# ivpml84079/Probabilistic-Self-Update-Line-Vector-Set-Based-Point-Cloud-Registration

Hardware: NVIDIA B200
Metric: registrations/s (higher is better)
Workload: dtype f64+f32

## Files before the change

probabilistic-self-update-line-vector-set-based-point-cloud-registration_b200/csrc/engine.cu:

```cuda
#include <cuda_runtime.h>
#include <sched.h>

#include <algorithm>
#include <atomic>
#include <chrono>
#if defined(__SSE2__)
#include <emmintrin.h>
#endif
#include <cmath>
#include <cstdlib>
#include <cstring>
#include <condition_variable>
#include <deque>
#include <functional>
#include <map>
#include <memory>
#include <mutex>
#include <string>
#include <thread>
#include <utility>
#include <vector>

#include "common.cuh"
#include "engine.cuh"
// ... 621 lines not shown
    PSU_CUDA(cudaEventRecord(ev_begin, st));
  }
  PSU_CUDA(cudaMemsetAsync(m.border, 0, sizeof(unsigned long long) * (size_t)B, st));
  PSU_CUDA(cudaMemsetAsync(m.n_done, 0, sizeof(int) * 4, st));
  PSU_CUDA(cudaMemcpyAsync(m.k1, k1.data(), sizeof(K1Job) * (size_t)B, cudaMemcpyHostToDevice, st));
  PSU_CUDA(cudaMemcpyAsync(m.cj, cj.data(), sizeof(CompactJob) * (size_t)B, cudaMemcpyHostToDevice, st));
  PSU_CUDA(cudaMemcpyAsync(m.pj, pj.data(), sizeof(PackJob) * (size_t)2 * B, cudaMemcpyHostToDevice, st));

  if (ratio) {
    if (int rc = ratio_count(st, rj, m.rj, maxC, [&](size_t bytes) -> void* { return d_hist.ensure(bytes) ? nullptr : d_hist.p; },
                             ev_m0, ev_m1))
      return rc;
    launches += 8;
  } else {
    {
      dim3 grid((unsigned)((maxC + 255) / 256), (unsigned)(2 * B));
      engine_pack_kernel<<<grid, 256, 0, st>>>(m.pj);
      PSU_CHECK_LAUNCH("engine_pack_kernel");
      ++launches;
    }
    PSU_CUDA(cudaEventRecord(ev_m0, st));
    if (!sharded || row_e > row_b)
      if (int rc = launch_consistency_mask(st, m.k1, B, maxC, sharded ? row_e - row_b : maxC, true)) return rc;
    PSU_CUDA(cudaEventRecord(ev_m1, st));
    ++launches;
    if (int rc = launch_compact_edges(st, m.cj, B, maxC, true, false, false)) return rc;
    ++launches;
  }
  if (int rc = h_small.ensure((sizeof(unsigned long long) + sizeof(int)) * (size_t)B + 64 + 66 * sizeof(unsigned long long)))
    return rc;
  unsigned long long* h_nedges = reinterpret_cast<unsigned long long*>(h_small.p);
  volatile int* h_done = reinterpret_cast<volatile int*>(reinterpret_cast<char*>(h_small.p) + sizeof(unsigned long long) * (size_t)B);
  unsigned long long* h_counts = reinterpret_cast<unsigned long long*>(
      reinterpret_cast<char*>(h_small.p) + align_up((sizeof(unsigned long long) + sizeof(int)) * (size_t)B + 16, 16));
  std::vector<unsigned long long> shard_off;
  if (sharded) {
    if (int rc = comm_allgather_u64(comm, st, m.n_edges, m.counts_all)) return rc;
    PSU_CUDA(cudaMemcpyAsync(h_counts, m.counts_all, sizeof(unsigned long long) * (size_t)comm_world(comm),
                             cudaMemcpyDeviceToHost, st));
    PSU_CUDA(cudaStreamSynchronize(st));
    shard_off.assign((size_t)comm_world(comm) + 1, 0ull);
    for (int r = 0; r < comm_world(comm); ++r) shard_off[(size_t)r + 1] = shard_off[(size_t)r] + h_counts[r];
    h_nedges[0] = shard_off.back();
    PSU_CUDA(cudaMemcpyAsync(m.n_edges, h_nedges, sizeof(unsigned long long), cudaMemcpyHostToDevice, st));
  } else {
    PSU_CUDA(cudaMemcpyAsync(h_nedges, m.n_edges, sizeof(unsigned long long) * (size_t)B, cudaMemcpyDeviceToHost, st));
    PSU_CUDA(cudaStreamSynchronize(st));
  }

  bool narrow = !sharded && !debug_knobs().edge_wide;
  for (int b = 0; b < B; ++b) narrow = narrow && edge_narrow_fits(lay[(size_t)(b0 + b)].Ccap);
  const int grid_ctas_max = sm_count() / (B > 0 ? B : 1);
  unsigned long long max_cap = 0, max_nred = 0;
  {
    Bump be;
    for (int pass = 0; pass < 2; ++pass) {
      be.off = 0;
      for (int b = 0; b < B; ++b) {
        JobCtl& J = jobs[(size_t)b];
        unsigned long long cap = h_nedges[b] + reserve[(size_t)(b0 + b)];
        if (cap < 64) cap = 64;
        J.edge_cap = cap;
        J.edges = narrow ? (void*)be.take<EdgeNarrow::T>((size_t)cap) : (void*)be.take<EdgeWide::T>((size_t)cap);
        J.first_words = sample_table_words(cap, sample_default_max_draws(cap, cap));
        J.first = be.take<uint32_t>((size_t)J.first_words);
        J.draws_cap = (cap + 3) & ~3ull;
        J.draws = be.take<uint32_t>((size_t)J.draws_cap);
        J.chunk_prefix = be.take<unsigned long long>((size_t)sample_chunk_slots(sample_default_max_draws(cap, cap)));
        J.ticket = be.take<unsigned int>(4);
        J.blist_cap = sample_list_entries(cap, cap) ? sample_list_entries(cap, cap) : 0ull;
        J.blist = J.blist_cap ? be.take<uint32_t>((size_t)J.blist_cap) : nullptr;
        J.bcount = be.take<unsigned int>((size_t)sample_list_counters());
        J.vbits = be.take<uint32_t>((size_t)((cap + 31) / 32 + 32));
        J.L_sampled = be.take<uint32_t>((size_t)cap);
        J.basic_idx = be.take<uint32_t>((size_t)cap);
        J.basic_edges = be.take<uint2>((size_t)cap);
        J.weights = be.take<double>((size_t)cap);
        J.lv_cap = cap / 6 + 64;
        J.lv = be.take<double>((size_t)6 * J.lv_cap);
        J.gnc_perm = be.take<uint32_t>((size_t)2 * J.lv_cap);
        if (grid_ctas_max >= 16) {
          J.gnc_grid_red = be.take<double>((size_t)grid_ctas_max * GNC_GRID_RED_DOUBLES);
          J.gnc_grid_bar = be.take<unsigned int>(4);
        }
        J.pruned_edges = ratio ? be.take<uint2>((size_t)cap) : nullptr;
        if (ratio) {
          rj[(size_t)b].edges = J.edges;
          rj[(size_t)b].cap = cap;
        }
        cj[(size_t)b].edges = static_cast<EdgeWide::T*>(J.edges) + (sharded && be.base ? shard_off[(size_t)comm_rank(comm)] : 0ull);
        cj[(size_t)b].cap = cap - (sharded ? shard_off[(size_t)comm_rank(comm)] : 0ull);
        max_cap = cap > max_cap ? cap : max_cap;
        max_nred = h_nedges[b] > max_nred ? h_nedges[b] : max_nred;
      }
      if (pass == 0) {
        if (int rc = d_edge.ensure(be.off)) return rc;
        be.base = reinterpret_cast<char*>(d_edge.p);
      }
    }
  }
  if (max_cap >= 0x7FFFFFF0ull) return fail(PSULVSB_ERR_UNSUPPORTED, "reduced set exceeds the 31-bit sample / line-vector indices");
  PSU_CUDA(cudaMemcpyAsync(m.jobs, jobs.data(), sizeof(JobCtl) * (size_t)B, cudaMemcpyHostToDevice, st));
  if (ratio) {
    if (int rc = ratio_emit(st, rj, m.rj, maxC, narrow)) return rc;
  } else {
    PSU_CUDA(cudaMemcpyAsync(m.cj, cj.data(), sizeof(CompactJob) * (size_t)B, cudaMemcpyHostToDevice, st));
    if (int rc = launch_compact_edges(st, m.cj, B, maxC, false, true, narrow)) return rc;
    if (sharded) {
      std::vector<unsigned long long> off32(shard_off);
      for (auto& o : off32) o *= 2ull;
      if (int rc = comm_allgatherv_inplace_u32(comm, st, reinterpret_cast<uint32_t*>(jobs[0].edges), off32.data())) return rc;
    }
  }
  ++launches;

  EngineParams P;
  P.caller = SubParams{params->noise_bound, params->cbar2, params->rotation_max_iterations, params->rotation_gnc_factor,
                       params->rotation_cost_threshold};
  P.inloop = SubParams{params->inloop_noise_bound, params->inloop_cbar2, params->inloop_max_iterations,
                       params->inloop_gnc_factor, params->inloop_cost_threshold};
  P.pr_noise = 2 * params->score_noise_bound;
  P.score_sigma = params->score_noise_bound;
  P.rotation_similar = params->rotation_similar;
  P.local_max_iter = params->local_max_iter;
  P.tpro_host = params->tpro_host;
// ... 667 lines not shown
```

probabilistic-self-update-line-vector-set-based-point-cloud-registration_b200/csrc/engine.cuh:

```cuda
#pragma once

#include <cuda_runtime.h>
#include <math.h>
#include <stdint.h>

#include <functional>
#include <vector>

#include "common.cuh"
#include "edge_fmt.cuh"

namespace psulvsb {

struct K1Consts {
  float half_bias;
  float two_beta2;
  float r0;
  float kappa;
  float w_thr;
  double beta;
  float beta4;
  float t_fast;
};
K1Consts make_k1_consts(double beta, double coord_bound);
// ... 111 lines not shown
  unsigned long long n_edges;
  const double* src;
  const double* dst;
  double beta;
  int filter;
  int n_vertices;
  uint32_t* adj;
  int stride;
  uint8_t* flags;
  int* size;
  int* proven;
  int active;
};
inline size_t clique_scratch_words(int n_vertices) {
  return (((size_t)n_vertices * (size_t)((n_vertices + 31) / 32) + 3) & ~(size_t)3) + 8;
}
int launch_max_clique(cudaStream_t st, const CliqueJob* d_jobs, int n_jobs, int max_vertices, int max_stride,
                      unsigned long long max_edges, bool exact);

int launch_knn_normals(cudaStream_t st, const double* pts, int n, int k, const double* viewpoint, double* normals);

int launch_pack_points(cudaStream_t st, const double* pts, int n, const double center[3], float4* out);
int launch_interleave_points(cudaStream_t st, const float4* in, int n, float4* out);
int launch_consistency_mask(cudaStream_t st, const K1Job* d_jobs, int n_jobs, int max_n, int max_rows, bool row_sectors);
int launch_symmetrize(cudaStream_t st, uint32_t* mask, int n, int stride);
int launch_compact_edges(cudaStream_t st, const CompactJob* d_jobs, int n_jobs, int max_n, bool scan, bool emit,
                         bool narrow);
int ratio_count(cudaStream_t st, std::vector<RatioJob>& rj, RatioJob* d_rj, int max_n,
                const std::function<void*(size_t)>& hist_arena, cudaEvent_t ev0, cudaEvent_t ev1);
int ratio_emit(cudaStream_t st, const std::vector<RatioJob>& rj, RatioJob* d_rj, int max_n, bool narrow);

__host__ __device__ inline unsigned long long sample_max_draws_formula(unsigned long long n,
                                                                       unsigned long long count) {
  if (n == 0 || count == 0) return 0;
  if (count > n) count = n;
  double e;
  if (count == n) {
    e = (double)n * (log((double)n) + 0.5772156649 + 10.0);
  } else {
    const double f = (double)count / (double)n;
    const double mean = -(double)n * log1p(-f);
    e = mean * 1.02 + 8.0 * sqrt(mean + 1.0) + 64.0;
  }
  unsigned long long m = (unsigned long long)e + 8;
  m = (m + 3) & ~3ull;
  if (m > 0xFFFFFFF0ull) m = 0xFFFFFFF0ull;
  return m;
}
unsigned long long sample_default_max_draws(unsigned long long n, unsigned long long count);
unsigned long long sample_chunk_slots(unsigned long long max_draws);
unsigned long long sample_list_entries(unsigned long long n, unsigned long long max_draws);
unsigned long long sample_list_counters();
unsigned long long sample_table_words(unsigned long long n, unsigned long long max_draws);
int launch_sample(cudaStream_t st, const SampleJob* d_jobs, int n_jobs, unsigned long long max_draws_bound,
                  unsigned long long n_bound, int flag_points = 0, bool narrow = false);
int launch_philox_fill(cudaStream_t st, uint64_t seed, uint32_t domain, uint32_t event, unsigned long long first_k,
                       unsigned long long count, uint32_t* out);

int gnc_default_capacity();
int gnc_cluster_for(int n_jobs);
int launch_gnc_tls(cudaStream_t st, const GncJob* d_jobs, int n_jobs, int cap_per_cta, int cluster, int n_active = 0);
int launch_kabsch_batch(cudaStream_t st, const double* src, const double* dst, const uint2* edges,
                        const uint32_t* sets, int k, unsigned long long n_hyp, double* R, double* t);

int launch_tls_translation(cudaStream_t st, const double* src, const double* dst, const uint8_t* flags, int n,
                           double scale, const double* R, double noise, const double* last_best, double* t_out,
                           int* n_points);
int launch_score_one(cudaStream_t st, const double* src, const double* dst, int n, double scale, const double* R,
                     const double* t, double tau, uint8_t* inliers, double* residuals, int* count);
int launch_score_batch(cudaStream_t st, const float4* src, const float4* dst, const double* src64, const double* dst64,
                       int n, const double* hyp, unsigned long long n_hyp, unsigned long long hyp_begin, double scale,
                       double tau, double coord_bound, const double* csrc, const double* cdst, uint32_t* counts,
                       unsigned long long* best, unsigned long long* border);

struct Comm;
int comm_unique_id(void* out128);
int comm_create(Comm** out, int device, int rank, int world, const void* id128);
void comm_destroy(Comm* c);
int comm_rank(const Comm* c);
int comm_world(const Comm* c);
int comm_allreduce_sum_u32(Comm* c, cudaStream_t st, uint32_t* d_inout, size_t n);
int comm_allreduce_max_u64(Comm* c, cudaStream_t st, unsigned long long* d_inout, size_t n);
int comm_allgather_u64(Comm* c, cudaStream_t st, const unsigned long long* d_send, unsigned long long* d_recv);
int comm_allgatherv_inplace_u32(Comm* c, cudaStream_t st, uint32_t* base, const unsigned long long* offsets);
void triangular_row_range(int n, int rank, int world, int* begin, int* end);

class EnginePool;
int pool_create(EnginePool** out, int device);
void pool_destroy(EnginePool* p);
int pool_set_batching(EnginePool* p, int chunk, int lanes);
int pool_set_host_threads(EnginePool* p, int n);
int pool_solve_one(EnginePool* p, const psulvsb_params_t* params, const psulvsb_problem_t* problem,
                   psulvsb_solution_t* solution, psulvsb_trace_t* trace);
int pool_solve_batch(EnginePool* p, const psulvsb_params_t* params, const psulvsb_problem_t* problems, int B,
                     const uint64_t* seeds, psulvsb_solution_t* solutions);
int pool_submit(EnginePool* p, const psulvsb_params_t* params, const psulvsb_problem_t* problems, int B,
                const uint64_t* seeds, psulvsb_solution_t* solutions, uint64_t* ticket);
int pool_wait(EnginePool* p, uint64_t ticket);
int pool_upload(EnginePool* p, const psulvsb_problem_t* problems, int B);
int pool_solve_sharded(EnginePool* p, Comm* comm, const psulvsb_params_t* params, const psulvsb_problem_t* problem,
                       psulvsb_solution_t* solution, psulvsb_trace_t* trace);
int pool_solve_resident(EnginePool* p, const psulvsb_params_t* params, const uint64_t* seeds,
                        psulvsb_solution_t* solutions, psulvsb_trace_t* trace_first);
int pool_batch_size(const EnginePool* p);
int pool_last_ticks(const EnginePool* p);
int pool_last_chunk_ticks(const EnginePool* p, int* out, int cap);
// ... 6 lines not shown
```

probabilistic-self-update-line-vector-set-based-point-cloud-registration_b200/csrc/engine_kernels.cu:

```cuda
#include <cuda_runtime.h>

#include "common.cuh"
#include "engine.cuh"
#include "engine_kernels.cuh"
#include "engine_state.cuh"
#include "solve_dev.cuh"
#include "svd3.cuh"

namespace psulvsb {

static_assert(kCtlThreads == BLK, "control kernels assume BLK threads");

namespace {

__device__ __constant__ double kLRate[4] = {0.1, 0.2, 0.5, 1.0};
__device__ __constant__ double kBRate[4] = {0.3, 0.3, 0.3, 1.0};

__device__ __forceinline__ void xform_identity(Xform& x) {
  x.s = 1.0;
#pragma unroll
  for (int i = 0; i < 9; ++i) x.R[i] = (i % 4 == 0) ? 1.0 : 0.0;
  x.t[0] = x.t[1] = x.t[2] = 0.0;
}

// ... 75 lines not shown
  q.dst = J.dst;
  q.beta = 2.0 * J.cur.noise_bound * sqrt(J.cur.cbar2);
  q.filter = 1;
  q.n_vertices = J.C;
  q.adj = J.adj;
  q.stride = J.adj_stride;
  q.flags = J.clique_flags;
  q.size = &J.clique_size;
  q.proven = &J.clique_proven;
}

__device__ int count_flagged(BlockScratch* s, const JobCtl& J, const Xform& X) {
  int cnt = 0, dummy = 0;
  for (int j = threadIdx.x; j < J.C; j += BLK)
    if (J.sampled_flags[j] && residual_ref(J.src + 3 * (size_t)j, J.dst + 3 * (size_t)j, X.s, X.R, X.t) <= J.tau) ++cnt;
  block_sum_int2(s, cnt, dummy);
  return cnt;
}

}

__global__ void __launch_bounds__(BLK)
    engine_init_kernel(JobCtl* __restrict__ jobs, SampleJob* __restrict__ sl, SampleJob* __restrict__ sb,
                       GncJob* __restrict__ gj, CliqueJob* __restrict__ cq,
                       const unsigned long long* __restrict__ n_edges, EngineParams P,
                       int* __restrict__ n_done) {
  JobCtl& J = jobs[blockIdx.x];
  const int tid = blockIdx.y * BLK + threadIdx.x;
  const int stride = gridDim.y * BLK;
  for (int i = tid; i < 3 * J.C0; i += stride) {
    J.src[i] = J.src0[i];
    J.dst[i] = J.dst0[i];
  }
  for (int i = tid; i < J.C0; i += stride) {
#pragma unroll
    for (int r = 0; r < 3; ++r) {
      J.pts8[8 * (size_t)i + r] = J.src0[3 * (size_t)i + r];
      J.pts8[8 * (size_t)i + 3 + r] = J.dst0[3 * (size_t)i + r];
    }
    J.pts8[8 * (size_t)i + 6] = 0.0;
    J.pts8[8 * (size_t)i + 7] = 0.0;
  }
  for (int j = tid; j < J.M; j += stride) {
    J.keep_mask[j] = J.keep_mask0[j];
    J.reduce_map[j] = J.reduce_map0[j];
    J.inlier_counter[j] = 0;
    J.new_corr[j] = 0;
    J.inlier_history[j] = -1;
    J.final_inliers[j] = 0;
    J.residual_history[j] = 0.0;
  }
  if (P.zero_sampler_scratch)
    for (unsigned long long i = tid; i < J.first_words; i += stride) J.first[i] = 0u;
  for (int i = tid; i < P.sampler_counters; i += stride) J.bcount[i] = 0u;
  if (P.zero_sampler_scratch)
    for (unsigned long long i = tid; i < (J.edge_cap + 31) / 32 + 32; i += stride) J.vbits[i] = 0u;
  if (tid == 0) {
    *J.ticket = 0u;
    J.C = J.C0;
    J.n_red0 = n_edges[blockIdx.x];
    J.n_red = J.n_red0;
    J.n_ls = 0;
    J.n_sampled_pts = 0;
    J.basic_choose = 0;
    J.phase = PHASE_ROUND_START;
    J.status = PSULVSB_OK;
    J.rounds_left = P.host_round_limit;
    J.host_round = 0;
    J.local_iter_global = 0;
    J.host_scorings = 0;
    J.escalations = 0;
    J.first_time = 1;
    J.sampled_first_time = 1;
    J.inloop = 0;
    J.longholi = 0;
    J.rate_idx = 0;
    J.local_r = 0;
    J.host_r = 0;
    J.best_sampled_cnt = 0;
    J.best_host_cnt = 0;
    J.pro_local = 0.0;
    J.pro_host = 0.0;
    J.pro_host_not_over = 1;
    J.scale_noise = 0.0;
    J.translation_noise = 0.0;
    xform_identity(J.sol);
    xform_identity(J.best_sampled);
    xform_identity(J.best_host);
    xform_identity(J.last_best);
    J.new_corr_count = 0;
    J.inlier_map_size = 0;
    J.scale_calls = 0;
    J.n_pruned = 0;
    J.cur_scale = 1.0;
    J.sample_status[0] = J.sample_status[1] = 1ull;
    J.n_local_trace = 0;
    J.n_host_trace = 0;
    J.valid = 0;
    J.refined = 0;
    sl[blockIdx.x].active = 0;
    sb[blockIdx.x].active = 0;
    gj[blockIdx.x].active = 0;
    cq[blockIdx.x].active = 0;
    J.clique_size = 0;
    J.aborted = 0;
    if (J.n_red0 > J.edge_cap) {
      J.status = PSULVSB_ERR_CAPACITY;
// ... 724 lines not shown
```

probabilistic-self-update-line-vector-set-based-point-cloud-registration_b200/csrc/k2_sampler.cu:

```cuda
#include <cstdlib>
#include <cuda_runtime.h>

#include "common.cuh"
#include "engine.cuh"

namespace psulvsb {

namespace {

constexpr int SMP_THREADS = 256;
constexpr int SMP_CHUNK = SMP_THREADS * 4;
constexpr int SMB_THREADS = 1024;
constexpr int SMP_BW = 49152;
constexpr int SMP_MAX_LIST_BUCKETS = 512;
constexpr int SMF_THREADS = 256;
constexpr int SMF_MAX_POINTS = 65536 * 8;

struct ListPlan {
  unsigned int n_buckets, w_bits, width;
  unsigned int wide;
  unsigned long long cap_b;
};
__host__ __device__ inline unsigned long long list_cap_for(unsigned long long n, unsigned long long max_draws,
                                                          unsigned long long width) {
  const unsigned long long mean = (max_draws * width + n - 1) / n + 1;
  unsigned long long s = 1;
  while (s * s < mean) ++s;
  return (mean + 10 * s + 64 + 3) & ~3ull;
}
__host__ __device__ inline bool sample_list_plan(unsigned long long n, unsigned long long max_draws,
                                                 unsigned long long blist_cap, ListPlan& p) {
  p.n_buckets = 0;
  p.cap_b = 0;
  p.wide = 0;
  if (max_draws < 2 || n < 3ull * SMP_BW) return false;
  unsigned int k_bits = 1;
  while (((max_draws - 1) >> k_bits) != 0ull) ++k_bits;
  if (k_bits <= 24) {
    p.w_bits = 32u - k_bits;
    p.width = (p.w_bits >= 16u) ? (unsigned int)SMP_BW : (1u << p.w_bits);
    const unsigned long long nb = (n + p.width - 1) / p.width;
    if (nb >= 3 && nb <= (unsigned long long)SMP_MAX_LIST_BUCKETS) {
      p.n_buckets = (unsigned int)nb;
      p.cap_b = list_cap_for(n, max_draws, p.width);
      if (nb * p.cap_b <= blist_cap) return true;
    }
  }
  if (k_bits > 32) return false;
  p.w_bits = 32u;
  p.width = (unsigned int)SMP_BW;
  const unsigned long long nbw = (n + SMP_BW - 1) / SMP_BW;
  if (nbw < 3 || nbw > (unsigned long long)SMP_MAX_LIST_BUCKETS) {
    p.n_buckets = 0;
    p.cap_b = 0;
    return false;
  }
  p.n_buckets = (unsigned int)nbw;
  p.cap_b = list_cap_for(n, max_draws, p.width);
  p.wide = 1;
  return 2ull * nbw * p.cap_b <= blist_cap;
}
__device__ __forceinline__ uint32_t list_bucket(uint32_t v, const ListPlan& p) {
  return (p.w_bits >= 16u) ? v / (uint32_t)SMP_BW : v >> p.w_bits;
}

struct FastMod {
  unsigned long long magic;
  uint32_t n;
};
__device__ __forceinline__ FastMod make_fastmod(uint32_t n) {
  FastMod f;
  f.n = n;
  f.magic = n > 1u ? (~0ull / n) + 1ull : 0ull;
  return f;
}
__device__ __forceinline__ uint32_t draw_value(uint32_t word, const FastMod& f) {
  const uint32_t v = word >> 1;
  if (f.n <= 1u) return 0u;
  const uint32_t q = (uint32_t)__umul64hi((unsigned long long)v, f.magic);
  return v - q * f.n;
}

__global__ void __launch_bounds__(256) sample_draws_kernel(const SampleJob* __restrict__ jobs, unsigned int list_cap_test) {
  const SampleJob& job = jobs[blockIdx.y];
  if (!job.active || job.identity) return;
  const bool cache = job.draws != nullptr && job.max_draws <= job.draws_cap;
  const unsigned long long nblocks = (job.max_draws + 3) >> 2;
  if ((unsigned long long)blockIdx.x * 256 >= nblocks) return;
  __shared__ ListPlan plan_s;
  __shared__ FastMod fm_s;
  __shared__ int lists_s;
  if (threadIdx.x == 0) {
    lists_s = (job.blist != nullptr && sample_list_plan(job.n, job.max_draws, job.blist_cap, plan_s)) ? 1 : 0;
    fm_s = make_fastmod((uint32_t)job.n);
  }
  __syncthreads();
  const ListPlan plan = plan_s;
  const bool lists = lists_s != 0;
  const unsigned int n_buckets = plan.n_buckets;
  const unsigned long long cap_b = plan.cap_b;
  const unsigned long long cap_fill = (list_cap_test != 0u && list_cap_test < plan.cap_b) ? list_cap_test : plan.cap_b;
  if (!cache && !lists) return;
  const FastMod fm = fm_s;
  uint4* __restrict__ out = reinterpret_cast<uint4*>(job.draws);
  if (!lists) {
    for (unsigned long long q = (unsigned long long)blockIdx.x * 256 + threadIdx.x; q < nblocks;
         q += (unsigned long long)gridDim.x * 256) {
      const Philox4 o = philox4x32_10(job.seed, job.domain, job.event, q);
      out[q] = make_uint4(draw_value(o.w[0], fm), draw_value(o.w[1], fm), draw_value(o.w[2], fm), draw_value(o.w[3], fm));
    }
    return;
  }
  constexpr int QPT = 4;
  __shared__ unsigned int wh[8][SMP_MAX_LIST_BUCKETS];
  __shared__ unsigned int base[SMP_MAX_LIST_BUCKETS];
  const int tid = threadIdx.x, lane = tid & 31, wid = tid >> 5;
  const unsigned int lt_mask = (1u << lane) - 1u;
  const unsigned long long max_draws = job.max_draws;
  for (unsigned long long q0 = (unsigned long long)blockIdx.x * (256 * QPT); q0 < nblocks;
       q0 += (unsigned long long)gridDim.x * (256 * QPT)) {
    uint32_t vv[QPT][4];
    unsigned int rk[QPT][4];
    for (int b = lane; b < (int)n_buckets; b += 32) wh[wid][b] = 0u;
#pragma unroll
    for (int u = 0; u < QPT; ++u) {
      const unsigned long long q = q0 + (unsigned long long)u * 256 + tid;
#pragma unroll
      for (int l = 0; l < 4; ++l) vv[u][l] = 0xFFFFFFFFu;
      if (q < nblocks) {
        const Philox4 o = philox4x32_10(job.seed, job.domain, job.event, q);
        uint32_t v4[4];
#pragma unroll
        for (int l = 0; l < 4; ++l) v4[l] = draw_value(o.w[l], fm);
        if (cache) out[q] = make_uint4(v4[0], v4[1], v4[2], v4[3]);
#pragma unroll
        for (int l = 0; l < 4; ++l)
          if ((q << 2) + l < max_draws) vv[u][l] = v4[l];
      }
    }
    __syncwarp();
#pragma unroll
    for (int u = 0; u < QPT; ++u)
#pragma unroll
      for (int l = 0; l < 4; ++l) {
        const uint32_t b = (vv[u][l] != 0xFFFFFFFFu) ? list_bucket(vv[u][l], plan) : 0xFFFFFFFFu;
        const unsigned int peers = __match_any_sync(0xffffffffu, b);
        const int leader = __ffs(peers) - 1;
        unsigned int start = 0u;
        if (lane == leader && b != 0xFFFFFFFFu) {
          start = wh[wid][b];
          wh[wid][b] = start + __popc(peers);
        }
        start = __shfl_sync(0xffffffffu, start, leader);
        rk[u][l] = start + __popc(peers & lt_mask);
        __syncwarp();
      }
    __syncthreads();
    for (int bk = tid; bk < (int)n_buckets; bk += 256) {
      unsigned int run = 0u;
#pragma unroll
      for (int w = 0; w < 8; ++w) {
        const unsigned int c = wh[w][bk];
        wh[w][bk] = run;
        run += c;
      }
      if (run != 0u) base[bk] = atomicAdd(&job.bcount[bk], run);
    }
    __syncthreads();
#pragma unroll
    for (int u = 0; u < QPT; ++u) {
      const unsigned long long q = q0 + (unsigned long long)u * 256 + tid;
#pragma unroll
      for (int l = 0; l < 4; ++l) {
        if (vv[u][l] == 0xFFFFFFFFu) continue;
        const uint32_t b = list_bucket(vv[u][l], plan);
        const unsigned long long pos = (unsigned long long)base[b] + wh[wid][b] + rk[u][l];
        if (pos < cap_fill) {
          if (plan.wide)
            reinterpret_cast<uint2*>(job.blist)[(unsigned long long)b * cap_b + pos] =
                make_uint2(vv[u][l] - b * plan.width, (uint32_t)((q << 2) + l));
          else
            job.blist[(unsigned long long)b * cap_b + pos] =
                (uint32_t)((((q << 2) + l) << plan.w_bits) | (unsigned long long)(vv[u][l] - b * plan.width));
        } else
          atomicExch(&job.bcount[SMP_MAX_LIST_BUCKETS], 1u);
      }
    }
    __syncthreads();
  }
}

__global__ void __launch_bounds__(SMB_THREADS, 1) sample_bucket_kernel(const SampleJob* __restrict__ jobs) {
  const SampleJob& job = jobs[blockIdx.y];
  if (!job.active) return;
  extern __shared__ __align__(16) unsigned char smem_raw[];
  uint32_t* table = reinterpret_cast<uint32_t*>(smem_raw);
  uint32_t* wbm = table + SMP_BW;
  __shared__ unsigned int ticket_s, sh[SMB_THREADS / 32];
  __shared__ unsigned long long carry_s;
  const int tid = threadIdx.x;
  if (job.post == 1 && blockIdx.x == 0)
    for (int i = tid; i < job.n_points; i += SMB_THREADS) job.flags[i] = 0;
  if (job.identity) return;
  const uint32_t n = (uint32_t)job.n;
  const FastMod fm = make_fastmod(n);
  ListPlan plan;
  const bool list_mode = job.blist != nullptr && sample_list_plan(job.n, job.max_draws, job.blist_cap, plan);
  const bool lists = list_mode && __ldcg(job.bcount + SMP_MAX_LIST_BUCKETS) == 0u;
  const unsigned int n_buckets = lists ? plan.n_buckets : (n + SMP_BW - 1) / SMP_BW;
  if (blockIdx.x >= n_buckets) return;
  const unsigned int n_workers = min(gridDim.x, n_buckets);
  const unsigned long long max_draws = job.max_draws;
  const unsigned long long nblocks = (max_draws + 3) >> 2;
  const bool cached = job.draws != nullptr && max_draws <= job.draws_cap;
  const uint4* __restrict__ dv = reinterpret_cast<const uint4*>(job.draws);
  uint32_t* __restrict__ accept = job.first;
  uint32_t* __restrict__ vbits = (job.post == 1) ? job.vbits : nullptr;
  auto draws_of = [&](uint32_t q) -> uint4 {
    if (cached) return __ldcg(dv + q);
    const Philox4 o = philox4x32_10(job.seed, job.domain, job.event, q);
    return make_uint4(draw_value(o.w[0], fm), draw_value(o.w[1], fm), draw_value(o.w[2], fm), draw_value(o.w[3], fm));
  };
  if (lists && plan.wide) {
    const uint2* __restrict__ lists2 = reinterpret_cast<const uint2*>(job.blist);
    for (uint32_t i = tid; i < plan.width; i += SMB_THREADS) table[i] = 0xFFFFFFFFu;
    for (unsigned int b = blockIdx.x; b < n_buckets; b += gridDim.x) {
      const uint2* __restrict__ list = lists2 + (unsigned long long)b * plan.cap_b;
      const uint32_t cnt = __ldcg(job.bcount + b);
      if (vbits)
        for (uint32_t i = tid; i < (plan.width >> 5); i += SMB_THREADS) wbm[i] = 0u;
      __syncthreads();
      for (uint32_t i = tid; i < cnt; i += SMB_THREADS) {
        const uint2 e = __ldcg(list + i);
        atomicMin(&table[e.x], e.y);
      }
      __syncthreads();
      const uint32_t lo_b = b * plan.width;
      for (uint32_t i = tid; i < cnt; i += SMB_THREADS) {
        const uint2 e = __ldcg(list + i);
        if (table[e.x] == e.y) {
          atomicOr(&accept[e.y >> 5], 1u << (e.y & 31));
          if (vbits) atomicOr(&wbm[e.x >> 5], 1u << (e.x & 31u));
        }
      }
      __syncthreads();
      if (vbits)
        for (uint32_t i = tid; i < (plan.width >> 5); i += SMB_THREADS)
          if (wbm[i] && ((unsigned long long)lo_b + 32ull * i) < job.n) vbits[(lo_b >> 5) + i] = wbm[i];
// ... 122 lines not shown
    if (vbits) {
      __syncthreads();
      for (uint32_t i = tid; i < ((width + 31u) >> 5); i += SMB_THREADS)
        if (wbm[i]) vbits[(lo >> 5) + i] = wbm[i];
    }
  }
  }
  __threadfence();
  __syncthreads();
  if (tid == 0) ticket_s = atomicAdd(job.ticket, 1u);
  __syncthreads();
  if (ticket_s != n_workers - 1) return;
  __threadfence();
  if (tid == 0) {
    carry_s = 0ull;
    *job.ticket = 0u;
    if (job.blist != nullptr) job.bcount[SMP_MAX_LIST_BUCKETS] = 0u;
  }
  __syncthreads();
  const unsigned long long nchunks = (max_draws + SMP_CHUNK - 1) / SMP_CHUNK;
  constexpr int WPC = SMP_CHUNK / 32;
  const unsigned long long nwords = (max_draws + 31) >> 5;
  for (unsigned long long c0 = 0; c0 < nchunks; c0 += SMB_THREADS) {
    const unsigned long long ch = c0 + tid;
    unsigned int v = 0;
    if (ch < nchunks)
      for (int w = 0; w < WPC; ++w) {
        const unsigned long long wi = ch * WPC + w;
        if (wi < nwords) v += __popc(__ldcg(accept + wi));
      }
    const int lane = tid & 31, wid = tid >> 5;
    unsigned int incl = v;
#pragma unroll
    for (int o = 1; o < 32; o <<= 1) {
      const unsigned int t = __shfl_up_sync(0xffffffffu, incl, o);
      if (lane >= o) incl += t;
    }
    if (lane == 31) sh[wid] = incl;
    __syncthreads();
    unsigned int wbase = 0;
#pragma unroll
    for (int w = 0; w < SMB_THREADS / 32; ++w)
      if (w < wid) wbase += sh[w];
    const unsigned long long carry = carry_s;
    if (ch < nchunks) job.chunk_prefix[ch] = carry + wbase + (incl - v);
    __syncthreads();
    if (tid == SMB_THREADS - 1) carry_s = carry + wbase + incl;
    __syncthreads();
  }
  if (tid == 0 && carry_s < job.count && job.status) job.status[0] = 0ull;
}

template <class F>
__global__ void __launch_bounds__(SMP_THREADS) sample_emit_kernel(const SampleJob* __restrict__ jobs) {
  const SampleJob& job = jobs[blockIdx.y];
  if (!job.active) return;
  __shared__ unsigned int sh[SMP_THREADS / 32];
  const int tid = threadIdx.x, lane = tid & 31, wid = tid >> 5;
  const unsigned long long count = job.count;
  uint32_t* __restrict__ out = job.out;
  if (job.identity) {
    for (unsigned long long r = (unsigned long long)blockIdx.x * SMP_THREADS + tid; r < count;
         r += (unsigned long long)gridDim.x * SMP_THREADS) {
      out[r] = (uint32_t)r;
      if (job.post == 1) {
        const uint2 e = F::load(job.edges, r);
        job.flags[e.x] = 1;
        job.flags[e.y] = 1;
      } else if (job.post == 2) {
        job.gathered[r] = F::load(job.edges, job.via[r]);
      }
    }
    if (blockIdx.x == 0 && tid == 0 && job.status) job.status[0] = 1ull;
    return;
  }
  const FastMod fm = make_fastmod((uint32_t)job.n);
  const unsigned long long max_draws = job.max_draws;
  const unsigned long long nchunks = (max_draws + SMP_CHUNK - 1) / SMP_CHUNK;
  const unsigned long long nwords = (max_draws + 31) >> 5;
  const bool cached = job.draws != nullptr && max_draws <= job.draws_cap;
  uint32_t* __restrict__ accept = job.first;
  for (unsigned long long ch = blockIdx.x; ch < nchunks; ch += gridDim.x) {
    const unsigned long long q = ch * SMP_THREADS + tid;
    const unsigned long long wi = q >> 3;
    const uint32_t word = (wi < nwords) ? __ldcg(accept + wi) : 0u;
    const uint32_t bits = (word >> ((q & 7) << 2)) & 0xFu;
    const unsigned int c = __popc(bits);
    unsigned int incl = c;
#pragma unroll
    for (int o = 1; o < 32; o <<= 1) {
      const unsigned int t = __shfl_up_sync(0xffffffffu, incl, o);
      if (lane >= o) incl += t;
    }
    if (lane == 31) sh[wid] = incl;
    __syncthreads();
    unsigned int wbase = 0;
#pragma unroll
    for (int w = 0; w < SMP_THREADS / 32; ++w)
      if (w < wid) wbase += sh[w];
    if ((q & 7) == 0 && wi < nwords && word != 0u) accept[wi] = 0u;
    unsigned long long rank = job.chunk_prefix[ch] + wbase + (incl - c);
    if (bits) {
      uint32_t vv[4];
      if (cached) {
        const uint4 d4 = __ldcg(reinterpret_cast<const uint4*>(job.draws) + q);
        vv[0] = d4.x; vv[1] = d4.y; vv[2] = d4.z; vv[3] = d4.w;
      } else {
        const Philox4 o = philox4x32_10(job.seed, job.domain, job.event, q);
#pragma unroll
        for (int l = 0; l < 4; ++l) vv[l] = draw_value(o.w[l], fm);
      }
#pragma unroll
      for (int l = 0; l < 4; ++l) {
        if ((bits >> l) & 1u) {
          if (rank < count) {
            const uint32_t v = vv[l];
            out[rank] = v;
            if (job.post == 1 && !job.vbits) {
              const uint2 e = F::load(job.edges, v);
              job.flags[e.x] = 1;
              job.flags[e.y] = 1;
            } else if (job.post == 2) {
              const uint2 e = F::load(job.edges, job.via[v]);
              job.gathered[rank] = e;
              if (job.lv_out && rank < job.lv_cap) {
                const double2* pa = reinterpret_cast<const double2*>(job.pts8 + 8 * (size_t)e.x);
                const double2* pb = reinterpret_cast<const double2*>(job.pts8 + 8 * (size_t)e.y);
                const double2 a0 = __ldg(pa), a1 = __ldg(pa + 1), a2 = __ldg(pa + 2);
                const double2 b0 = __ldg(pb), b1 = __ldg(pb + 1), b2 = __ldg(pb + 2);
                double* __restrict__ o = job.lv_out + rank;
                const size_t st = (size_t)job.lv_cap;
                __stcg(o, b0.x - a0.x);
                __stcg(o + st, b0.y - a0.y);
                __stcg(o + 2 * st, b1.x - a1.x);
                __stcg(o + 3 * st, b1.y - a1.y);
                __stcg(o + 4 * st, b2.x - a2.x);
                __stcg(o + 5 * st, b2.y - a2.y);
              }
            }
            if (rank == count - 1 && job.status) job.status[0] = (q << 2) + l + 1;
          } else if (job.post == 1 && job.vbits) {
            atomicAnd(&job.vbits[vv[l] >> 5], ~(1u << (vv[l] & 31u)));
          }
          ++rank;
        }
      }
    }
    __syncthreads();
  }
}

template <class F>
__global__ void __launch_bounds__(SMF_THREADS) sample_flag_kernel(const SampleJob* __restrict__ jobs, int onchip_points) {
  const SampleJob& job = jobs[blockIdx.y];
  if (!job.active || job.identity || job.post != 1 || !job.vbits) return;
  extern __shared__ uint32_t pbits[];
  const int tid = threadIdx.x;
  const bool onchip = job.n_points <= onchip_points;
  const int pwords = (job.n_points + 31) >> 5;
  if (onchip) {
    for (int i = tid; i < pwords; i += SMF_THREADS) pbits[i] = 0u;
    __syncthreads();
  }
  uint8_t* __restrict__ flags = job.flags;
  auto mark = [&](uint32_t p) {
    if (!onchip) {
      flags[p] = 1;
      return;
    }
    const uint32_t bit = 1u << (p & 31u);
    if (!(pbits[p >> 5] & bit)) atomicOr(&pbits[p >> 5], bit);
  };
  const unsigned long long nwords = (job.n + 31) >> 5;
  const unsigned long long threads = (unsigned long long)gridDim.x * SMF_THREADS;
  const void* __restrict__ edges = job.edges;
  for (unsigned long long wi = (unsigned long long)blockIdx.x * SMF_THREADS + tid; wi < nwords; wi += threads) {
    uint32_t word = __ldcg(job.vbits + wi);
    if (!word) continue;
    job.vbits[wi] = 0u;
    const unsigned long long row = wi * 32;
    while (word) {
      uint2 e[4];
      int m = 0;
#pragma unroll
      for (int j = 0; j < 4; ++j) {
        if (word) {
          const int bit = __ffs(word) - 1;
          word &= word - 1;
          e[j] = F::load(edges, row + bit);
          m = j + 1;
        }
// ... 10 lines not shown
  __syncthreads();
  for (int w = tid; w < pwords; w += SMF_THREADS) {
    const uint32_t bits = pbits[w];
    if (!bits) continue;
    uint8_t* __restrict__ f = flags + 32 * (size_t)w;
#pragma unroll
    for (int h = 0; h < 2; ++h) {
      const uint32_t half = (bits >> (16 * h)) & 0xFFFFu;
      if (half == 0xFFFFu) {
        reinterpret_cast<uint4*>(f)[h] = make_uint4(0x01010101u, 0x01010101u, 0x01010101u, 0x01010101u);
        continue;
      }
#pragma unroll
      for (int q = 0; q < 4; ++q) {
        const uint32_t nib = (half >> (4 * q)) & 0xFu;
        uint8_t* __restrict__ g = f + 16 * h + 4 * q;
        if (nib == 0xFu)
          *reinterpret_cast<uint32_t*>(g) = 0x01010101u;
        else
#pragma unroll
          for (int l = 0; l < 4; ++l)
            if ((nib >> l) & 1u) g[l] = 1;
      }
    }
  }
}

__global__ void philox_fill_kernel(uint64_t seed, uint32_t domain, uint32_t event, unsigned long long first_k,
                                   unsigned long long count, uint32_t* __restrict__ out) {
  const unsigned long long i = (unsigned long long)blockIdx.x * blockDim.x + threadIdx.x;
  if (i < count) out[i] = philox_rand31(seed, domain, event, first_k + i);
}

}

unsigned long long sample_default_max_draws(unsigned long long n, unsigned long long count) {
  return sample_max_draws_formula(n, count);
}

unsigned long long sample_list_entries(unsigned long long n, unsigned long long max_draws) {
  ListPlan p;
  if (!sample_list_plan(n, max_draws, ~0ull, p)) return 0;
  return (unsigned long long)p.n_buckets * p.cap_b * (p.wide ? 2ull : 1ull);
}
unsigned long long sample_list_counters() { return SMP_MAX_LIST_BUCKETS + 4; }

unsigned long long sample_chunk_slots(unsigned long long max_draws) { return (max_draws + SMP_CHUNK - 1) / SMP_CHUNK + 1; }

unsigned long long sample_table_words(unsigned long long n, unsigned long long max_draws) {
  (void)n;
  return (max_draws + 31) / 32 + 8;
}

int launch_sample(cudaStream_t st, const SampleJob* d_jobs, int n_jobs, unsigned long long max_draws_bound,
                  unsigned long long n_bound, int flag_points, bool narrow) {
  if (n_jobs <= 0) return PSULVSB_OK;
  static bool attr_set = false;
  const size_t smem = (size_t)SMP_BW * 4 + (size_t)SMP_BW / 8;
  const int fsmem_max = SMF_MAX_POINTS / 8;
  if (!attr_set) {
    PSU_CUDA(cudaFuncSetAttribute(sample_bucket_kernel, cudaFuncAttributeMaxDynamicSharedMemorySize, (int)smem));
    PSU_CUDA(cudaFuncSetAttribute(sample_flag_kernel<EdgeWide>, cudaFuncAttributeMaxDynamicSharedMemorySize, fsmem_max));
    PSU_CUDA(cudaFuncSetAttribute(sample_flag_kernel<EdgeNarrow>, cudaFuncAttributeMaxDynamicSharedMemorySize, fsmem_max));
    attr_set = true;
  }
  const unsigned long long nchunks = (max_draws_bound + SMP_CHUNK - 1) / SMP_CHUNK;
  unsigned long long gx = nchunks;
  const unsigned long long cap = (unsigned long long)(sm_count() * 16) / (unsigned long long)(n_jobs < 64 ? n_jobs : 64) + 1;
  if (gx > cap) gx = cap;
  if (gx < 1) gx = 1;
  const unsigned int list_cap_test = (unsigned int)debug_knobs().sample_list_cap_test;
  sample_draws_kernel<<<dim3((unsigned)gx, (unsigned)n_jobs), 256, 0, st>>>(d_jobs, list_cap_test);
  PSU_CHECK_LAUNCH("sample_draws_kernel");
  unsigned long long nb = (n_bound + SMP_BW - 1) / SMP_BW;
  if (nb < 1) nb = 1;
  unsigned long long bx = ((unsigned long long)sm_count() * 3ull + (unsigned long long)n_jobs - 1) / (unsigned long long)n_jobs;
  if (bx > nb) bx = nb;
  if (bx < 1) bx = 1;
  sample_bucket_kernel<<<dim3((unsigned)bx, (unsigned)n_jobs), SMB_THREADS, smem, st>>>(d_jobs);
  PSU_CHECK_LAUNCH("sample_bucket_kernel");
  if (narrow)
    sample_emit_kernel<EdgeNarrow><<<dim3((unsigned)gx, (unsigned)n_jobs), SMP_THREADS, 0, st>>>(d_jobs);
  else
    sample_emit_kernel<EdgeWide><<<dim3((unsigned)gx, (unsigned)n_jobs), SMP_THREADS, 0, st>>>(d_jobs);
  PSU_CHECK_LAUNCH("sample_emit_kernel");
  if (flag_points > 0) {
    unsigned long long fx = (n_bound + 32ull * SMF_THREADS - 1) / (32ull * SMF_THREADS);
    const unsigned long long fcap = ((unsigned long long)sm_count() * 16 + (unsigned long long)n_jobs - 1) / (unsigned long long)n_jobs;
    if (fx > fcap) fx = fcap;
    if (fx < 1) fx = 1;
    const int onchip_points = flag_points <= SMF_MAX_POINTS ? flag_points : 0;
    const size_t fsmem = (size_t)(onchip_points + 31) / 32 * 4;
    if (narrow)
      sample_flag_kernel<EdgeNarrow><<<dim3((unsigned)fx, (unsigned)n_jobs), SMF_THREADS, fsmem, st>>>(d_jobs, onchip_points);
    else
      sample_flag_kernel<EdgeWide><<<dim3((unsigned)fx, (unsigned)n_jobs), SMF_THREADS, fsmem, st>>>(d_jobs, onchip_points);
    PSU_CHECK_LAUNCH("sample_flag_kernel");
  }
  return PSULVSB_OK;
}

int launch_philox_fill(cudaStream_t st, uint64_t seed, uint32_t domain, uint32_t event, unsigned long long first_k,
                       unsigned long long count, uint32_t* out) {
  if (count == 0) return PSULVSB_OK;
  philox_fill_kernel<<<(unsigned)((count + 255) / 256), 256, 0, st>>>(seed, domain, event, first_k, count, out);
  PSU_CHECK_LAUNCH("philox_fill_kernel");
  return PSULVSB_OK;
}

}
```

Before: 16020.

## Add single-CTA on-chip sampling walk for small edge sets

For jobs with at most about a million candidates, sampling without replacement now runs inside one CTA of the bucket kernel. It keeps a shared-memory seen bitmap and a small hash table that settles duplicate draws by lowest draw index, with a serial warp fallback when there are too many collisions. This skips the global draws cache and bucket lists and drops their allocation and zeroing. The trade is that one CTA per job does the whole sequential walk, which can lower parallelism on large samples, and the draws and emit kernels still launch but exit early.

```diff
diff --git a/probabilistic-self-update-line-vector-set-based-point-cloud-registration_b200/csrc/engine.cu b/probabilistic-self-update-line-vector-set-based-point-cloud-registration_b200/csrc/engine.cu
--- a/probabilistic-self-update-line-vector-set-based-point-cloud-registration_b200/csrc/engine.cu
+++ b/probabilistic-self-update-line-vector-set-based-point-cloud-registration_b200/csrc/engine.cu
@@ -697,6 +697,9 @@
   for (int b = 0; b < B; ++b) narrow = narrow && edge_narrow_fits(lay[(size_t)(b0 + b)].Ccap);
   const int grid_ctas_max = sm_count() / (B > 0 ? B : 1);
   unsigned long long max_cap = 0, max_nred = 0;
+  bool sample_onchip = true;
+  for (int b = 0; b < B; ++b)
+    sample_onchip = sample_onchip && sample_onchip_bound(std::max(h_nedges[b] + reserve[(size_t)(b0 + b)], 64ull));
   {
     Bump be;
     for (int pass = 0; pass < 2; ++pass) {
@@ -709,13 +712,13 @@
         J.edges = narrow ? (void*)be.take<EdgeNarrow::T>((size_t)cap) : (void*)be.take<EdgeWide::T>((size_t)cap);
         J.first_words = sample_table_words(cap, sample_default_max_draws(cap, cap));
         J.first = be.take<uint32_t>((size_t)J.first_words);
-        J.draws_cap = (cap + 3) & ~3ull;
-        J.draws = be.take<uint32_t>((size_t)J.draws_cap);
+        J.draws_cap = sample_onchip ? 0ull : (cap + 3) & ~3ull;
+        J.draws = J.draws_cap ? be.take<uint32_t>((size_t)J.draws_cap) : nullptr;
         J.chunk_prefix = be.take<unsigned long long>((size_t)sample_chunk_slots(sample_default_max_draws(cap, cap)));
         J.ticket = be.take<unsigned int>(4);
-        J.blist_cap = sample_list_entries(cap, cap) ? sample_list_entries(cap, cap) : 0ull;
+        J.blist_cap = sample_onchip ? 0ull : sample_list_entries(cap, cap);
         J.blist = J.blist_cap ? be.take<uint32_t>((size_t)J.blist_cap) : nullptr;
-        J.bcount = be.take<unsigned int>((size_t)sample_list_counters());
+        J.bcount = J.blist ? be.take<unsigned int>((size_t)sample_list_counters()) : nullptr;
         J.vbits = be.take<uint32_t>((size_t)((cap + 31) / 32 + 32));
         J.L_sampled = be.take<uint32_t>((size_t)cap);
         J.basic_idx = be.take<uint32_t>((size_t)cap);
diff --git a/probabilistic-self-update-line-vector-set-based-point-cloud-registration_b200/csrc/engine.cuh b/probabilistic-self-update-line-vector-set-based-point-cloud-registration_b200/csrc/engine.cuh
--- a/probabilistic-self-update-line-vector-set-based-point-cloud-registration_b200/csrc/engine.cuh
+++ b/probabilistic-self-update-line-vector-set-based-point-cloud-registration_b200/csrc/engine.cuh
@@ -187,6 +187,7 @@
 unsigned long long sample_list_entries(unsigned long long n, unsigned long long max_draws);
 unsigned long long sample_list_counters();
 unsigned long long sample_table_words(unsigned long long n, unsigned long long max_draws);
+bool sample_onchip_bound(unsigned long long n_bound);
 int launch_sample(cudaStream_t st, const SampleJob* d_jobs, int n_jobs, unsigned long long max_draws_bound,
                   unsigned long long n_bound, int flag_points = 0, bool narrow = false);
 int launch_philox_fill(cudaStream_t st, uint64_t seed, uint32_t domain, uint32_t event, unsigned long long first_k,
diff --git a/probabilistic-self-update-line-vector-set-based-point-cloud-registration_b200/csrc/engine_kernels.cu b/probabilistic-self-update-line-vector-set-based-point-cloud-registration_b200/csrc/engine_kernels.cu
--- a/probabilistic-self-update-line-vector-set-based-point-cloud-registration_b200/csrc/engine_kernels.cu
+++ b/probabilistic-self-update-line-vector-set-based-point-cloud-registration_b200/csrc/engine_kernels.cu
@@ -151,7 +151,8 @@
   }
   if (P.zero_sampler_scratch)
     for (unsigned long long i = tid; i < J.first_words; i += stride) J.first[i] = 0u;
-  for (int i = tid; i < P.sampler_counters; i += stride) J.bcount[i] = 0u;
+  if (J.bcount)
+    for (int i = tid; i < P.sampler_counters; i += stride) J.bcount[i] = 0u;
   if (P.zero_sampler_scratch)
     for (unsigned long long i = tid; i < (J.edge_cap + 31) / 32 + 32; i += stride) J.vbits[i] = 0u;
   if (tid == 0) {
diff --git a/probabilistic-self-update-line-vector-set-based-point-cloud-registration_b200/csrc/k2_sampler.cu b/probabilistic-self-update-line-vector-set-based-point-cloud-registration_b200/csrc/k2_sampler.cu
--- a/probabilistic-self-update-line-vector-set-based-point-cloud-registration_b200/csrc/k2_sampler.cu
+++ b/probabilistic-self-update-line-vector-set-based-point-cloud-registration_b200/csrc/k2_sampler.cu
@@ -15,6 +15,11 @@
 constexpr int SMP_MAX_LIST_BUCKETS = 512;
 constexpr int SMF_THREADS = 256;
 constexpr int SMF_MAX_POINTS = 65536 * 8;
+constexpr int SMO_CHUNK = SMB_THREADS * 4;
+constexpr int SMO_HASH = 4096;
+constexpr unsigned int SMO_LOSE_CAP = SMO_HASH / 2;
+constexpr unsigned long long SMO_MAX_N = 1ull << 20;
+constexpr unsigned long long SMO_MAX_DRAWS = 1ull << 20;
 
 struct ListPlan {
   unsigned int n_buckets, w_bits, width;
@@ -81,9 +86,160 @@
   return v - q * f.n;
 }
 
-__global__ void __launch_bounds__(256) sample_draws_kernel(const SampleJob* __restrict__ jobs, unsigned int list_cap_test) {
+__host__ __device__ inline bool sample_onchip(const SampleJob& job, unsigned long long onchip_n) {
+  return job.n <= onchip_n && job.max_draws <= SMO_MAX_DRAWS && !job.identity && (job.post != 1 || job.vbits != nullptr);
+}
+
+__device__ __forceinline__ uint32_t philox_word(const Philox4& o, uint32_t l) {
+  return l == 0u ? o.w[0] : l == 1u ? o.w[1] : l == 2u ? o.w[2] : o.w[3];
+}
+
+__device__ __forceinline__ uint32_t onchip_hash(uint32_t v) { return (v * 0x9E3779B1u) >> (32 - 12); }
+
+__device__ void sample_onchip_walk(const SampleJob& job, uint32_t* __restrict__ smem, unsigned int lose_cap) {
+  constexpr uint32_t EMPTY = 0xFFFFFFFFu;
+  uint32_t* seen = smem;
+  uint32_t* hkey = smem + SMO_MAX_N / 32;
+  uint32_t* hmin = hkey + SMO_HASH;
+  __shared__ unsigned int n_lose_s;
+  __shared__ unsigned int wsum[SMB_THREADS / 32];
+  __shared__ uint32_t walk_acc[SMO_CHUNK / 32];
+  const int tid = threadIdx.x, lane = tid & 31, wid = tid >> 5;
+  const uint32_t n = (uint32_t)job.n;
+  const uint32_t nwords = (n + 31u) >> 5;
+  for (uint32_t i = tid; i < nwords; i += SMB_THREADS) seen[i] = 0u;
+  for (int i = tid; i < SMO_HASH; i += SMB_THREADS) hkey[i] = EMPTY;
+  if (job.post == 1)
+    for (int i = tid; i < job.n_points; i += SMB_THREADS) job.flags[i] = 0;
+  if (tid == 0) n_lose_s = 0u;
+  const FastMod fm = make_fastmod(n);
+  const uint64_t seed = job.seed;
+  const uint32_t domain = job.domain, event = job.event;
+  const uint32_t md = (uint32_t)job.max_draws, cnt = (uint32_t)job.count;
+  uint32_t* __restrict__ out = job.out;
+  uint32_t taken = 0u;
+  __syncthreads();
+  for (uint32_t k0 = 0u; k0 < md && taken < cnt; k0 += SMO_CHUNK) {
+    const uint32_t kt = k0 + 4u * (uint32_t)tid;
+    const Philox4 o = philox4x32_10(seed, domain, event, kt >> 2);
+    uint32_t v[4];
+    unsigned int acc = 0u;
+#pragma unroll
+    for (int l = 0; l < 4; ++l) {
+      v[l] = draw_value(o.w[l], fm);
+      if (kt + l < md && !((seen[v[l] >> 5] >> (v[l] & 31u)) & 1u)) acc |= 1u << l;
+    }
+    __syncthreads();
+    int slot[4];
+#pragma unroll
+    for (int l = 0; l < 4; ++l) {
+      slot[l] = -1;
+      if ((acc >> l) & 1u) {
+        const uint32_t bit = 1u << (v[l] & 31u);
+        if ((atomicOr(&seen[v[l] >> 5], bit) & bit) && atomicAdd(&n_lose_s, 1u) < lose_cap) {
+          uint32_t h = onchip_hash(v[l]);
+          while (true) {
+            const uint32_t old = atomicCAS(&hkey[h], EMPTY, v[l]);
+            if (old == EMPTY) hmin[h] = 0xFFFFFFFFu;
+            if (old == EMPTY || old == v[l]) break;
+            h = (h + 1u) & (SMO_HASH - 1u);
+          }
+          slot[l] = (int)h;
+        }
+      }
+    }
+    __syncthreads();
+    const unsigned int n_lose = n_lose_s;
+    if (n_lose > lose_cap) {
+#pragma unroll
+      for (int l = 0; l < 4; ++l) {
+        if (slot[l] >= 0) hkey[slot[l]] = EMPTY;
+        if ((acc >> l) & 1u) atomicAnd(&seen[v[l] >> 5], ~(1u << (v[l] & 31u)));
+      }
+      __syncthreads();
+      if (wid == 0)
+        for (uint32_t j = 0; j < (uint32_t)SMO_CHUNK; j += 32u) {
+          const uint32_t k = k0 + j + lane;
+          const uint32_t vk = draw_value(philox_word(philox4x32_10(seed, domain, event, k >> 2), k & 3u), fm);
+          const bool c = k < md && !((seen[vk >> 5] >> (vk & 31u)) & 1u);
+          const unsigned int peers = __match_any_sync(0xffffffffu, c ? vk : EMPTY);
+          const bool first = c && (__ffs(peers) - 1) == lane;
+          if (first) atomicOr(&seen[vk >> 5], 1u << (vk & 31u));
+          const unsigned int b = __ballot_sync(0xffffffffu, first);
+          if (lane == 0) walk_acc[j >> 5] = b;
+          __syncwarp();
+        }
+      __syncthreads();
+      acc = (walk_acc[(4u * tid) >> 5] >> ((4u * tid) & 31u)) & 0xFu;
+    } else if (n_lose > 0u) {
+#pragma unroll
+      for (int l = 0; l < 4; ++l)
+        if ((acc >> l) & 1u) {
+          if (slot[l] < 0) {
+            uint32_t h = onchip_hash(v[l]);
+            for (uint32_t key = hkey[h]; key != EMPTY; key = hkey[h]) {
+              if (key == v[l]) {
+                slot[l] = (int)h;
+                break;
+              }
+              h = (h + 1u) & (SMO_HASH - 1u);
+            }
+          }
+          if (slot[l] >= 0) atomicMin(&hmin[slot[l]], kt + l);
+        }
+      __syncthreads();
+#pragma unroll
+      for (int l = 0; l < 4; ++l)
+        if (slot[l] >= 0) {
+          if (hmin[slot[l]] != kt + l) acc &= ~(1u << l);
+          hkey[slot[l]] = EMPTY;
+        }
+    }
+    const unsigned int c = __popc(acc);
+    unsigned int incl = c;
+#pragma unroll
+    for (int d = 1; d < 32; d <<= 1) {
+      const unsigned int t = __shfl_up_sync(0xffffffffu, incl, d);
+      if (lane >= d) incl += t;
+    }
+    if (lane == 31) wsum[wid] = incl;
+    __syncthreads();
+    unsigned int wbase = 0u, total = 0u;
+#pragma unroll
+    for (int w = 0; w < SMB_THREADS / 32; ++w) {
+      const unsigned int s = wsum[w];
+      wbase += (w < wid) ? s : 0u;
+      total += s;
+    }
+    if (tid == 0) n_lose_s = 0u;
+    uint32_t rank = taken + wbase + (incl - c);
+#pragma unroll
+    for (int l = 0; l < 4; ++l)
+      if ((acc >> l) & 1u) {
+        if (rank < cnt) {
+          out[rank] = v[l];
+          if (rank == cnt - 1u && job.status) job.status[0] = (unsigned long long)(kt + l) + 1ull;
+        } else {
+          atomicAnd(&seen[v[l] >> 5], ~(1u << (v[l] & 31u)));
+        }
+        ++rank;
+      }
+    taken += total;
+  }
+  if (tid == 0 && taken < cnt && job.status) job.status[0] = 0ull;
+  if (job.post == 1) {
+    __syncthreads();
+    for (uint32_t i = tid; i < nwords; i += SMB_THREADS) {
+      const uint32_t w = seen[i];
+      if (w) job.vbits[i] = w;
+    }
+  }
+}
+
+__global__ void __launch_bounds__(256) sample_draws_kernel(const SampleJob* __restrict__ jobs, unsigned int list_cap_test,
+                                                           unsigned long long onchip_n) {
   const SampleJob& job = jobs[blockIdx.y];
-  if (!job.active || job.identity) return;
+  if (!job.active || job.identity || sample_onchip(job, onchip_n)) return;
   const bool cache = job.draws != nullptr && job.max_draws <= job.draws_cap;
   const unsigned long long nblocks = (job.max_draws + 3) >> 2;
   if ((unsigned long long)blockIdx.x * 256 >= nblocks) return;
@@ -190,10 +346,15 @@
   }
 }
 
-__global__ void __launch_bounds__(SMB_THREADS, 1) sample_bucket_kernel(const SampleJob* __restrict__ jobs) {
+__global__ void __launch_bounds__(SMB_THREADS, 1) sample_bucket_kernel(const SampleJob* __restrict__ jobs,
+                                                                      unsigned long long onchip_n, unsigned int lose_cap) {
   const SampleJob& job = jobs[blockIdx.y];
   if (!job.active) return;
   extern __shared__ __align__(16) unsigned char smem_raw[];
+  if (sample_onchip(job, onchip_n)) {
+    if (blockIdx.x == 0) sample_onchip_walk(job, reinterpret_cast<uint32_t*>(smem_raw), lose_cap);
+    return;
+  }
   uint32_t* table = reinterpret_cast<uint32_t*>(smem_raw);
   uint32_t* wbm = table + SMP_BW;
   __shared__ unsigned int ticket_s, sh[SMB_THREADS / 32];
@@ -422,13 +583,41 @@
 }
 
 template <class F>
-__global__ void __launch_bounds__(SMP_THREADS) sample_emit_kernel(const SampleJob* __restrict__ jobs) {
+__device__ __forceinline__ void gather_basic(const SampleJob& job, unsigned long long rank, uint32_t v) {
+  const uint2 e = F::load(job.edges, job.via[v]);
+  job.gathered[rank] = e;
+  if (job.lv_out && rank < job.lv_cap) {
+    const double2* pa = reinterpret_cast<const double2*>(job.pts8 + 8 * (size_t)e.x);
+    const double2* pb = reinterpret_cast<const double2*>(job.pts8 + 8 * (size_t)e.y);
+    const double2 a0 = __ldg(pa), a1 = __ldg(pa + 1), a2 = __ldg(pa + 2);
+    const double2 b0 = __ldg(pb), b1 = __ldg(pb + 1), b2 = __ldg(pb + 2);
+    double* __restrict__ o = job.lv_out + rank;
+    const size_t st = (size_t)job.lv_cap;
+    __stcg(o, b0.x - a0.x);
+    __stcg(o + st, b0.y - a0.y);
+    __stcg(o + 2 * st, b1.x - a1.x);
+    __stcg(o + 3 * st, b1.y - a1.y);
+    __stcg(o + 4 * st, b2.x - a2.x);
+    __stcg(o + 5 * st, b2.y - a2.y);
+  }
+}
+
+template <class F>
+__global__ void __launch_bounds__(SMP_THREADS) sample_emit_kernel(const SampleJob* __restrict__ jobs,
+                                                                  unsigned long long onchip_n) {
   const SampleJob& job = jobs[blockIdx.y];
   if (!job.active) return;
   __shared__ unsigned int sh[SMP_THREADS / 32];
   const int tid = threadIdx.x, lane = tid & 31, wid = tid >> 5;
   const unsigned long long count = job.count;
   uint32_t* __restrict__ out = job.out;
+  if (sample_onchip(job, onchip_n)) {
+    if (job.post != 2 || (job.status && __ldcg(job.status) == 0ull)) return;
+    for (unsigned long long r = (unsigned long long)blockIdx.x * SMP_THREADS + tid; r < count;
+         r += (unsigned long long)gridDim.x * SMP_THREADS)
+      gather_basic<F>(job, r, __ldcg(out + r));
+    return;
+  }
   if (job.identity) {
     for (unsigned long long r = (unsigned long long)blockIdx.x * SMP_THREADS + tid; r < count;
          r += (unsigned long long)gridDim.x * SMP_THREADS) {
@@ -491,22 +680,7 @@
               job.flags[e.x] = 1;
               job.flags[e.y] = 1;
             } else if (job.post == 2) {
-              const uint2 e = F::load(job.edges, job.via[v]);
-              job.gathered[rank] = e;
-              if (job.lv_out && rank < job.lv_cap) {
-                const double2* pa = reinterpret_cast<const double2*>(job.pts8 + 8 * (size_t)e.x);
-                const double2* pb = reinterpret_cast<const double2*>(job.pts8 + 8 * (size_t)e.y);
-                const double2 a0 = __ldg(pa), a1 = __ldg(pa + 1), a2 = __ldg(pa + 2);
-                const double2 b0 = __ldg(pb), b1 = __ldg(pb + 1), b2 = __ldg(pb + 2);
-                double* __restrict__ o = job.lv_out + rank;
-                const size_t st = (size_t)job.lv_cap;
-                __stcg(o, b0.x - a0.x);
-                __stcg(o + st, b0.y - a0.y);
-                __stcg(o + 2 * st, b1.x - a1.x);
-                __stcg(o + 3 * st, b1.y - a1.y);
-                __stcg(o + 4 * st, b2.x - a2.x);
-                __stcg(o + 5 * st, b2.y - a2.y);
-              }
+              gather_basic<F>(job, rank, v);
             }
             if (rank == count - 1 && job.status) job.status[0] = (q << 2) + l + 1;
           } else if (job.post == 1 && job.vbits) {
@@ -623,11 +797,14 @@
   return (max_draws + 31) / 32 + 8;
 }
 
+bool sample_onchip_bound(unsigned long long n_bound) { return n_bound <= SMO_MAX_N; }
+
 int launch_sample(cudaStream_t st, const SampleJob* d_jobs, int n_jobs, unsigned long long max_draws_bound,
                   unsigned long long n_bound, int flag_points, bool narrow) {
   if (n_jobs <= 0) return PSULVSB_OK;
   static bool attr_set = false;
   const size_t smem = (size_t)SMP_BW * 4 + (size_t)SMP_BW / 8;
+  static_assert(SMO_MAX_N / 8 + 8 * SMO_HASH <= (size_t)SMP_BW * 4 + SMP_BW / 8, "the on-chip walk shares the bucket pass's shared memory");
   const int fsmem_max = SMF_MAX_POINTS / 8;
   if (!attr_set) {
     PSU_CUDA(cudaFuncSetAttribute(sample_bucket_kernel, cudaFuncAttributeMaxDynamicSharedMemorySize, (int)smem));
@@ -641,19 +818,21 @@
   if (gx > cap) gx = cap;
   if (gx < 1) gx = 1;
   const unsigned int list_cap_test = (unsigned int)debug_knobs().sample_list_cap_test;
-  sample_draws_kernel<<<dim3((unsigned)gx, (unsigned)n_jobs), 256, 0, st>>>(d_jobs, list_cap_test);
+  const unsigned long long onchip_n = sample_onchip_bound(n_bound) ? n_bound : 0ull;
+  const unsigned int lose_cap = (list_cap_test != 0u && list_cap_test < SMO_LOSE_CAP) ? list_cap_test : SMO_LOSE_CAP;
+  sample_draws_kernel<<<dim3((unsigned)gx, (unsigned)n_jobs), 256, 0, st>>>(d_jobs, list_cap_test, onchip_n);
   PSU_CHECK_LAUNCH("sample_draws_kernel");
   unsigned long long nb = (n_bound + SMP_BW - 1) / SMP_BW;
   if (nb < 1) nb = 1;
   unsigned long long bx = ((unsigned long long)sm_count() * 3ull + (unsigned long long)n_jobs - 1) / (unsigned long long)n_jobs;
   if (bx > nb) bx = nb;
   if (bx < 1) bx = 1;
-  sample_bucket_kernel<<<dim3((unsigned)bx, (unsigned)n_jobs), SMB_THREADS, smem, st>>>(d_jobs);
+  sample_bucket_kernel<<<dim3((unsigned)bx, (unsigned)n_jobs), SMB_THREADS, smem, st>>>(d_jobs, onchip_n, lose_cap);
   PSU_CHECK_LAUNCH("sample_bucket_kernel");
   if (narrow)
-    sample_emit_kernel<EdgeNarrow><<<dim3((unsigned)gx, (unsigned)n_jobs), SMP_THREADS, 0, st>>>(d_jobs);
+    sample_emit_kernel<EdgeNarrow><<<dim3((unsigned)gx, (unsigned)n_jobs), SMP_THREADS, 0, st>>>(d_jobs, onchip_n);
   else
-    sample_emit_kernel<EdgeWide><<<dim3((unsigned)gx, (unsigned)n_jobs), SMP_THREADS, 0, st>>>(d_jobs);
+    sample_emit_kernel<EdgeWide><<<dim3((unsigned)gx, (unsigned)n_jobs), SMP_THREADS, 0, st>>>(d_jobs, onchip_n);
   PSU_CHECK_LAUNCH("sample_emit_kernel");
   if (flag_points > 0) {
     unsigned long long fx = (n_bound + 32ull * SMF_THREADS - 1) / (32ull * SMF_THREADS);
```

After: 18660, median of 6. 1.16x the previous value.
